# scrubbbbs/cbird

Measured on AMD Instinct MI355X. Metric: Hamming comparisons/sec + images hashed/sec, 1M-image index, 1/2/4/8 MI355X, higher is better.
Workload: dtype u64 hashes as 64 x FP4 signs, f32 accumulate (find, exact) / u8+f32 (hash)

## Files before the change

cbird_amd/csrc/hamm64_mfma.hip:

```cpp
#include <algorithm>
#include <mutex>
#include <vector>

#include "cbh_internal.h"
#include "fp4_sign.h"

namespace cbh {
namespace {

typedef _Float16 h2 __attribute__((ext_vector_type(2)));
typedef unsigned v4u_t __attribute__((ext_vector_type(4)));

constexpr int kThreads = 256;
constexpr int kWaves = 4;
constexpr int kHT = 8;
constexpr int kG = 2;
constexpr int e8m0(int e) { return (int)((uint32_t)(127 + e) * 0x01010101u); }

constexpr uint32_t kNeedlePad = 384;
constexpr uint32_t kNeedleBytes = 80;
struct NeedleScratch {
  uint32_t nq_pad;
  __host__ __device__ constexpr uint32_t words() const { return 0u; }
  __host__ __device__ constexpr uint32_t fold() const { return 2u * nq_pad; }
  __host__ __device__ constexpr uint32_t pre48() const { return 3u * nq_pad; }
  __host__ __device__ constexpr uint32_t pre16() const { return pre48() + nq_pad / 128u * 192u; }
  __host__ __device__ constexpr uint32_t total() const { return pre16() + nq_pad / 128u * 64u; }
};
static_assert(kNeedlePad % 64u == 0 && kNeedlePad % 96u == 0 && kNeedlePad % 128u == 0,
              "whole pairs, triples and quadruples of needle tiles");
static_assert(NeedleScratch{kNeedlePad}.total() * 16u == kNeedlePad * kNeedleBytes &&
                  NeedleScratch{5u * kNeedlePad}.total() * 16u == 5u * kNeedlePad * kNeedleBytes,
              "the regions add up to kNeedleBytes per padded needle");

__global__ __launch_bounds__(256) void k_expand_needles(const uint64_t* __restrict__ q, uint32_t nq,
                                                        uint32_t nq_pad, uint4* __restrict__ qx) {
  const uint32_t i = blockIdx.x * 256u + threadIdx.x;
  const NeedleScratch L{nq_pad};
  if (i >= L.total()) return;
  const uint32_t* w = reinterpret_cast<const uint32_t*>(q);
  if (i < L.fold()) {
    qx[i] = fp4_expand32((i >> 1) < nq ? w[i] : 0u);
  } else if (i < L.pre48()) {
    const uint32_t j = i - L.fold();
    qx[i] = fp4_expand32(j < nq ? w[2u * j] ^ w[2u * j + 1u] : 0u);
  } else if (i < L.pre16()) {
    const uint32_t u = i - L.pre48(), quad = u / 192u, m = (u % 192u) >> 6, c = u & 31u, kb = (u >> 5) & 1u;
    uint2 o[2];
#pragma unroll
    for (uint32_t k = 0; k < 2; ++k) {
      const uint32_t s = 2u * (2u * m + kb) + k, j = quad * 128u + (s / 3u) * 32u + c;
      const uint32_t lo = j < nq ? w[2u * j] : 0u, hi = j < nq ? w[2u * j + 1u] : 0u;
      o[k] = fp4_expand16(pre48_sub(lo, hi, s % 3u), s == 3u || s == 7u || s == 9u ? kFp4Four : kFp4Half);
    }
    qx[i] = make_uint4(o[0].x, o[0].y, o[1].x, o[1].y);
  } else {
    const uint32_t u = i - L.pre16(), c = u & 31u, kb = (u >> 5) & 1u;
    const uint32_t j0 = (u >> 6) * 128u + kb * 64u + c, j1 = j0 + 32u;
    const uint2 lo = fp4_expand16(j0 < nq ? fold16(w[2u * j0], w[2u * j0 + 1u]) : 0u, kFp4Half);
    const uint2 hi = fp4_expand16(j1 < nq ? fold16(w[2u * j1], w[2u * j1 + 1u]) : 0u, kFp4Four);
    qx[i] = make_uint4(lo.x, lo.y, hi.x, hi.y);
  }
}

__device__ __forceinline__ uint32_t as_u32(float f) { return __builtin_bit_cast(uint32_t, f); }
__device__ __forceinline__ void wave_order() {
  asm volatile("" ::: "memory");
  __builtin_amdgcn_wave_barrier();
  asm volatile("" ::: "memory");
}
__device__ __forceinline__ uint32_t wave_rank(uint64_t m, uint32_t base = 0u) {
  return __builtin_amdgcn_mbcnt_hi((uint32_t)(m >> 32), __builtin_amdgcn_mbcnt_lo((uint32_t)m, base));
}
__device__ __forceinline__ uint32_t cd_row(uint32_t g, uint32_t lane) { return (g & 3u) + 8u * (g >> 2) + 4u * (lane >> 5); }

struct HitParams {
  uint32_t thresh, n, nq, keep0;
  const uint64_t* q;
  const uint32_t* ids;
  cbh_record* rec;
  unsigned long long cap;
  unsigned long long* total;
  const uint2* hay;
  const uint2* qmask;
};

constexpr uint32_t kOutCap = 128;
__device__ __forceinline__ void out_flush(uint32_t* s_out, uint32_t& nout, const HitParams& hp) {
  if (nout == 0) return;
  wave_order();
  const uint32_t lane = threadIdx.x & 63u;
  unsigned long long base = 0;
  if (lane == 0) base = atomicAdd(hp.total, (unsigned long long)nout);
  const uint32_t blo = (uint32_t)__builtin_amdgcn_readfirstlane((int)(uint32_t)base);
  const uint32_t bhi = (uint32_t)__builtin_amdgcn_readfirstlane((int)(uint32_t)(base >> 32));
  base = ((unsigned long long)bhi << 32) | blo;
  for (uint32_t k = lane; k < nout; k += 64u) {
    const uint2 r = *reinterpret_cast<const uint2*>(&s_out[2u * k]);
    if (base + k < hp.cap) hp.rec[base + k] = ((cbh_record)r.y << 32) | r.x;
  }
  wave_order();
  nout = 0;
}
__device__ __forceinline__ void out_push(uint32_t* s_out, uint32_t& nout, bool has, uint32_t qidx, uint32_t dist,
                                         uint32_t id, const HitParams& hp) {
  const uint64_t m = __builtin_amdgcn_ballot_w64(has);
  if (m == 0) return;
  const uint32_t c = (uint32_t)__popcll(m);
  if (nout + c > kOutCap) out_flush(s_out, nout, hp);
  if (has) *reinterpret_cast<uint2*>(&s_out[2u * wave_rank(m, nout)]) = make_uint2(id, (qidx << 7) | dist);
  nout += c;
}

__device__ __forceinline__ bool mask_ok(const HitParams& hp, uint32_t row, uint32_t qi, uint64_t nv) {
  if (!hp.qmask) return true;
  const uint2 hv = hp.hay[row], mk = hp.qmask[qi];
  return (((hv.x ^ (uint32_t)nv) & mk.x) | ((hv.y ^ (uint32_t)(nv >> 32)) & mk.y)) == 0;
}
__device__ __forceinline__ void out_match(uint32_t* s_out, uint32_t& nout, bool under, uint32_t row, uint32_t qi,
                                          uint64_t nv, uint32_t dist, const HitParams& hp) {
  bool has = false;
  uint32_t id = 0;
  if (under && row < hp.n && mask_ok(hp, row, qi, nv)) {
    id = hp.ids[row];
    has = id != 0 || hp.keep0;
  }
  out_push(s_out, nout, has, qi, dist, id, hp);
}

template <int N, class Step>
__device__ __forceinline__ void needle_loop(const uint4* base, uint32_t voff, uint32_t nsteps, uint32_t last, Step&& step) {
  const __amdgpu_buffer_rsrc_t rsrc = __builtin_amdgcn_make_buffer_rsrc(const_cast<uint4*>(base), 0, (int)0xffffffffu, 0x27000);
  auto load = [&](uint32_t s, uint4 (&o)[N]) __attribute__((always_inline)) {
#pragma unroll
    for (uint32_t m = 0; m < (uint32_t)N; ++m) {
      const v4u_t v = __builtin_amdgcn_raw_buffer_load_b128(rsrc, (int)voff, (int)(min(s * N + m, last) * 1024u), 0);
      o[m] = make_uint4(v.x, v.y, v.z, v.w);
    }
  };
  uint4 x[N], y[N];
  load(0, x);
#pragma unroll 1
  for (uint32_t s = 0; s < nsteps; s += 2) {
    load(min(s + 1, nsteps - 1), y);
    step(s, x);
    if (s + 1 < nsteps) {
      load(min(s + 2, nsteps - 1), x);
      step(s + 1, y);
    }
  }
}
constexpr uint32_t kNoClamp = 0xffffffffu;

constexpr uint32_t kFlagMaskPre = (1u << 5) | (1u << 11) | (1u << 17) | (1u << 23);
constexpr uint32_t kFieldOnes = 1u + (1u << 6) + (1u << 12) + (1u << 18);

constexpr uint32_t kPendCap = 320;
constexpr uint32_t kOutOff = 2u * kPendCap;
constexpr uint32_t kItemOff = kOutOff + 2u * kOutCap;
constexpr uint32_t kItemCap = 63u + 64u * 8u;
constexpr uint32_t kPreQueue = kItemOff + kItemCap + 1u;
static_assert(kPendCap >= 63u + (kHT / kG) * 64u, "pending list: every lane of every group of a step");
static_assert(kG == 2, "a descriptor names the two reduction chains of a group of 32 registers");

template <int A, int B, int G>
__device__ __forceinline__ uint32_t or_regs(const v16f (&c)[G]) {
  static_assert(B - A >= 3, "range");
  uint32_t o = as_u32(c[A >> 4][A & 15]) | as_u32(c[(A + 1) >> 4][(A + 1) & 15]) | as_u32(c[(A + 2) >> 4][(A + 2) & 15]);
#pragma unroll
  for (int r = A + 3; r < B; r += 2)
    o |= as_u32(c[r >> 4][r & 15]) | (r + 1 < B ? as_u32(c[(r + 1) >> 4][(r + 1) & 15]) : 0u);
  return o;
}

#define CBH_SCALED_MFMA(A, B, C, SCALE_B) __builtin_amdgcn_mfma_scale_f32_32x32x64_f8f6f4(A, B, C, 4, 4, 0, kScaleOne, 0, SCALE_B)

struct Pre32 {
  static constexpr int kTiles = kHT, kOps = 2;
  static constexpr uint32_t operands(NeedleScratch L) { return L.fold(); }
  static __device__ __forceinline__ uint32_t last_op(uint32_t n_pairs, uint32_t p0) { return n_pairs - 1u - p0; }
  static __device__ __forceinline__ v8i hay(uint2 hv, uint32_t) { return fp4_operand(fp4_expand32(hv.x ^ hv.y)); }
  static __device__ __forceinline__ uint32_t bias(uint32_t t) { return 16u + (t - 1u); }
  static __device__ __forceinline__ int scale(int m, uint32_t half) {
    return m == 0 ? (half ? e8m0(5) : e8m0(-1)) : (half ? e8m0(17) : e8m0(11));
  }
  static __device__ __forceinline__ void chain(const v8i (&a)[kTiles], int t0, const v8i (&b)[kOps], const v16f& c0,
                                               const int (&sc)[kOps], v16f (&c)[kG]) {
#pragma unroll
    for (int t = 0; t < kG; ++t) c[t] = CBH_SCALED_MFMA(a[t0 + t], b[0], c0, sc[0]);
#pragma unroll
    for (int t = 0; t < kG; ++t) c[t] = CBH_SCALED_MFMA(a[t0 + t], b[1], c[t], sc[1]);
  }
};

struct Pre48 {
  static constexpr int kTiles = 6, kOps = 3;
  static constexpr uint32_t operands(NeedleScratch L) { return L.pre48(); }
  static __device__ __forceinline__ uint32_t last_op(uint32_t, uint32_t) { return kNoClamp; }
  static __device__ __forceinline__ v8i hay(uint2 hv, uint32_t half) {
    const uint32_t e0 = pre48_sub(hv.x, hv.y, 0), e1 = pre48_sub(hv.x, hv.y, 1), e2 = pre48_sub(hv.x, hv.y, 2);
    const uint2 s0 = fp4_expand16(half ? e2 : e0, kFp4Half);
    const uint2 s1 = fp4_expand16(half ? e0 : e1, half ? kFp4Four : kFp4Half);
    const uint2 s2 = fp4_expand16(half ? e1 : e2, kFp4Half);
    const uint2 s3 = fp4_expand16(half ? e2 : e0, half ? kFp4Half : kFp4Four);
    return v8i{(int)s0.x, (int)s0.y, (int)s1.x, (int)s1.y, (int)s2.x, (int)s2.y, (int)s3.x, (int)s3.y};
  }
  static __device__ __forceinline__ uint32_t bias(uint32_t t) { return 8u + t; }
  static __device__ __forceinline__ int scale(int m, uint32_t half) {
    return m == 0 ? e8m0(1) : m == 1 ? (half ? e8m0(10) : e8m0(7)) : (half ? e8m0(19) : e8m0(13));
  }
  static __device__ __forceinline__ void chain(const v8i (&a)[kTiles], int t0, const v8i (&b)[kOps], const v16f& c0,
                                               const int (&sc)[kOps], v16f (&c)[kG]) {
#pragma unroll
    for (int m = 0; m < kOps; ++m)
#pragma unroll
      for (int t = 0; t < kG; ++t) {
        const v8i& h = a[t0 + t];
        c[t] = CBH_SCALED_MFMA((v8i{h[2 * m], h[2 * m + 1], h[2 * m + 2], h[2 * m + 3], 0, 0, 0, 0}), b[m], m ? c[t] : c0, sc[m]);
      }
  }
};

struct Pre16 {
  static constexpr int kTiles = kHT, kOps = 1;
  static constexpr uint32_t operands(NeedleScratch L) { return L.pre16(); }
  static __device__ __forceinline__ uint32_t last_op(uint32_t, uint32_t) { return kNoClamp; }
  static __device__ __forceinline__ v8i hay(uint2 hv, uint32_t) {
    const uint32_t f = fold16(hv.x, hv.y);
    const uint2 s0 = fp4_expand16(f, kFp4Half), s1 = fp4_expand16(f, kFp4Four);
    return v8i{(int)s0.x, (int)s0.y, (int)s1.x, (int)s1.y, 0, 0, 0, 0};
  }
  static __device__ __forceinline__ uint32_t bias(uint32_t t) { return 24u + (t - 1u); }
  static __device__ __forceinline__ int scale(int, uint32_t half) { return half ? e8m0(13) : e8m0(1); }
  static __device__ __forceinline__ void chain(const v8i (&a)[kTiles], int t0, const v8i (&b)[kOps], const v16f& c0,
                                               const int (&sc)[kOps], v16f (&c)[kG]) {
#pragma unroll
    for (int t = 0; t < kG; ++t) c[t] = CBH_SCALED_MFMA(a[t0 + t], b[0], c0, sc[0]);
  }
};

#define CBH_MFMA_PARAMS                                                                                              \
  const uint2 *__restrict__ hay, const uint32_t *__restrict__ ids, uint32_t n, const uint64_t *__restrict__ q,       \
      const uint4 *__restrict__ qx, uint32_t nq, uint32_t n_pairs, uint32_t pairs_per_chunk, uint32_t thresh,        \
      cbh_record *__restrict__ rec, unsigned long long cap, unsigned long long *__restrict__ total, uint32_t keep0,  \
      const uint2 *__restrict__ qmask, const uint4 *__restrict__ qf
#define CBH_MFMA_ARGS hay, ids, n, q, qx, nq, n_pairs, pairs_per_chunk, thresh, rec, cap, total, keep0, qmask, qf

template <class V>
__device__ __forceinline__ void prefilter_body(CBH_MFMA_PARAMS) {
  constexpr int HT = V::kTiles, G = kG;
  __shared__ __attribute__((aligned(16))) uint32_t s_queue_[kWaves][kPreQueue];
  __shared__ __attribute__((aligned(16))) uint2 s_hay_[kWaves][HT * 32];
  const uint32_t lane = threadIdx.x & 63u;
  const uint32_t wave = (uint32_t)__builtin_amdgcn_readfirstlane((int)(threadIdx.x >> 6));
  const uint32_t r = lane & 31u, half = lane >> 5;
  const uint32_t tile0 = (blockIdx.x * kWaves + wave) * HT;
  if (tile0 * 32u >= n) return;
  uint32_t* s_queue = s_queue_[wave];
  uint2* s_hay = s_hay_[wave];
  uint32_t* s_out = s_queue + kOutOff;
  uint32_t nout = 0;

  v8i a[HT];
#pragma unroll
  for (int t = 0; t < HT; ++t) {
    const uint32_t row = (tile0 + t) * 32u + r;
    const uint2 hv = row < n ? hay[row] : make_uint2(0u, 0u);
    a[t] = V::hay(hv, half);
    if (half == 0) s_hay[t * 32 + r] = hv;
  }
  wave_order();
  v16f c0;
#pragma unroll
  for (int g = 0; g < 16; ++g) c0[g] = 8388608.0f + (float)(V::bias(thresh) * kFieldOnes);
  asm volatile("" : "+v"(c0));
  int scale[V::kOps];
#pragma unroll
  for (int m = 0; m < V::kOps; ++m) {
    scale[m] = V::scale(m, half);
    asm volatile("" : "+v"(scale[m]));
  }

  const uint32_t p0 = blockIdx.y * pairs_per_chunk;
  const uint32_t p1 = min(n_pairs, p0 + pairs_per_chunk);
  const HitParams hp = {thresh, n, nq, keep0, q, ids, rec, cap, total, hay, qmask};

  uint32_t npend = 0;
  uint32_t nitem = 0;
  uint32_t* s_item = s_queue + kItemOff;
  auto work = [&](uint32_t idx, bool live) {
    const uint32_t it = s_item[idx];
    const uint32_t f = it & 3u, ch = (it >> 2) & 1u, L = (it >> 3) & 63u, pp = p0 + 2u * (it >> 11);
    const uint32_t row0 = ((it >> 9) & 3u) * 64u;
    const uint32_t qi = pp * 64u + (L & 31u) + 32u * f;
    const uint64_t nv = live && qi < hp.nq ? hp.q[qi] : 0;
    const uint32_t qlo = (uint32_t)nv, qhi = (uint32_t)(nv >> 32);
    const uint32_t rows = nv == 0 ? 0u : ch ? 0xfffe0000u : 0x0001ffffu;
    const uint2* hq = s_hay + row0 + cd_row(16u * ch, L);
    uint32_t hit = 0;
#pragma unroll 1
    for (uint32_t i = 0; i < 5u; ++i) {
      const uint32_t qd = 4u * ch + i;
      const uint4* h4 = reinterpret_cast<const uint4*>(hq + 8u * min(i, 4u - ch));
      const uint4 x = h4[0], y = h4[1];
      const uint32_t d0 = __popc(x.x ^ qlo) + __popc(x.y ^ qhi), d1 = __popc(x.z ^ qlo) + __popc(x.w ^ qhi);
      const uint32_t d2 = __popc(y.x ^ qlo) + __popc(y.y ^ qhi), d3 = __popc(y.z ^ qlo) + __popc(y.w ^ qhi);
      const uint32_t m4 = (d0 < hp.thresh ? 1u : 0u) | (d1 < hp.thresh ? 2u : 0u) | (d2 < hp.thresh ? 4u : 0u) |
                          (d3 < hp.thresh ? 8u : 0u);
      hit |= qd < 8u ? m4 << (4u * qd) : 0u;
    }
    hit &= rows;
    while (__builtin_amdgcn_ballot_w64(hit != 0) != 0) {
      const uint32_t wr = row0 + cd_row((uint32_t)__builtin_ctz(hit | 0x80000000u), L);
      const uint2 hv = s_hay[wr];
      out_match(s_out, nout, hit != 0, tile0 * 32u + wr, qi, nv, __popc(hv.x ^ qlo) + __popc(hv.y ^ qhi), hp);
      hit &= hit - 1u;
    }
  };
  auto drain = [&](bool all) {
    wave_order();
    const uint32_t keep = all ? 0u : (npend & 63u);
    uint32_t k0 = keep;
    for (;;) {
      if (nitem < 64u && k0 < npend) {
        const uint2 e = *reinterpret_cast<const uint2*>(&s_queue[2u * min(k0 + lane, npend - 1u)]);
        uint32_t cm = 0;
#pragma unroll
        for (uint32_t c = 0; c < 2; ++c) {
          const uint32_t w = e.x >> c;
          cm |= (((w >> 23) & 1u) ? 0xfu : (((w >> 5) & 1u) | (((w >> 11) & 1u) << 1) | (((w >> 17) & 1u) << 2))) << (4u * c);
        }
        if (k0 + lane >= npend) cm = 0;
#pragma unroll
        for (uint32_t b = 0; b < 8; ++b) {
          const bool on = ((cm >> b) & 1u) != 0;
          const uint64_t m = __builtin_amdgcn_ballot_w64(on);
          if (on) s_item[wave_rank(m, nitem)] = (e.y << 3) | b;
          nitem += (uint32_t)__popcll(m);
        }
        k0 += 64u;
        wave_order();
        continue;
      }
      uint32_t idx;
      bool live = true;
      if (nitem >= 64u) {
        nitem -= 64u;
        idx = nitem + lane;
      } else if (all && nitem != 0) {
        idx = min(lane, nitem - 1u);
        live = lane < nitem;
        nitem = 0;
      } else {
        break;
      }
      work(idx, live);
      wave_order();
    }
    npend = keep;
  };

  auto detect = [&](const v16f (&c)[G], const uint32_t group, const uint32_t step) __attribute__((always_inline)) {
    constexpr int R = G * 16;
    constexpr int RA = R / 2 + 1;
    const uint32_t half0 = or_regs<0, RA, G>(c), half1 = or_regs<RA, R, G>(c);
    const uint32_t flags = (half0 | half1) & kFlagMaskPre;
    const uint64_t hm = __builtin_amdgcn_ballot_w64(flags != 0);
    if (hm != 0) {
      static_assert(R == 32, "two chains of 17 and 15 registers");
      uint32_t ln = lane;
      asm volatile("" : "+v"(ln));
      if (flags != 0)
        *reinterpret_cast<uint2*>(&s_queue[2u * wave_rank(hm, npend)]) =
            make_uint2((half0 & kFlagMaskPre) | ((half1 & kFlagMaskPre) << 1), ln | (group << 6) | (step << 8));
      npend += (uint32_t)__popcll(hm);
    }
  };

  needle_loop<V::kOps>(qf + (size_t)(p0 >> 1) * (V::kOps * 64u), lane * 16u, (p1 - p0 + 1u) >> 1, V::last_op(n_pairs, p0),
                       [&](const uint32_t s, const uint4 (&nn)[V::kOps]) __attribute__((always_inline)) {
    v8i b[V::kOps];
#pragma unroll
    for (int m = 0; m < V::kOps; ++m) b[m] = fp4_operand(nn[m]);
#pragma unroll
    for (int t0 = 0; t0 < HT; t0 += G) {
      v16f c[G];
      V::chain(a, t0, b, c0, scale, c);
      detect(c, (uint32_t)(t0 / G), s);
    }
    if (npend >= 64u) drain(false);
  });
  if (npend | nitem) drain(true);
  out_flush(s_out, nout, hp);
}

template <bool PRE>
__global__ void k_hamm64_mfma(CBH_MFMA_PARAMS);
template <>
__global__ __launch_bounds__(kThreads, 4) void k_hamm64_mfma<true>(CBH_MFMA_PARAMS) { prefilter_body<Pre32>(CBH_MFMA_ARGS); }
__global__ __launch_bounds__(kThreads, 3) void k_hamm64_mfma48(CBH_MFMA_PARAMS) { prefilter_body<Pre48>(CBH_MFMA_ARGS); }
__global__ __launch_bounds__(kThreads, 4) void k_hamm64_mfma16(CBH_MFMA_PARAMS) { prefilter_body<Pre16>(CBH_MFMA_ARGS); }

__device__ __forceinline__ void load_hay_words(const uint2* __restrict__ hay, uint32_t n, uint32_t tile0, v8i (&a)[kHT]) {
  const uint32_t r = threadIdx.x & 31u, half = (threadIdx.x >> 5) & 1u;
#pragma unroll
  for (int t = 0; t < kHT; ++t) {
    const uint32_t row = (tile0 + t) * 32u + r;
    const uint2 hv = row < n ? hay[row] : make_uint2(0u, 0u);
    a[t] = fp4_operand(fp4_expand32(half ? hv.y : hv.x));
  }
}

constexpr uint32_t kLoZero2 = 0x4080u, kHiZero2 = 0x4B40u;
__device__ __forceinline__ h2 as_h2(float f) { return __builtin_bit_cast(h2, f); }
__device__ __forceinline__ h2 pkmax3(h2 a, h2 b, h2 c) {
  return __builtin_elementwise_maximum(__builtin_elementwise_maximum(a, b), c);
}
__device__ __forceinline__ void handle_tile2(const v16f& c, uint32_t row0, uint32_t p, uint32_t lo_key, uint32_t hi_key,
                                             const HitParams& hp, uint32_t* s_queue, uint32_t* s_out, uint32_t& nout) {
  const uint32_t lane = threadIdx.x & 63u;
  {
    h2 m0 = {0, 0}, m1 = {0, 0};
#pragma unroll
    for (int g = 0; g < 16; g += 4) {
      m0 = pkmax3(m0, as_h2(c[g]), as_h2(c[g + 1]));
      m1 = pkmax3(m1, as_h2(c[g + 2]), as_h2(c[g + 3]));
    }
    const uint32_t tb = __builtin_bit_cast(uint32_t, __builtin_elementwise_maximum(m0, m1));
    if (__builtin_amdgcn_ballot_w64((tb << 16) >= lo_key || tb >= hi_key) == 0) return;
  }
  uint32_t cnt = 0;
#pragma unroll
  for (int g = 0; g < 16; ++g) {
    const uint32_t bits = as_u32(c[g]);
    const bool fh = bits >= hi_key;
    const bool fl = (bits << 16) >= lo_key;
    if (__builtin_amdgcn_ballot_w64(fh || fl) == 0) continue;
    const uint64_t mh = __builtin_amdgcn_ballot_w64(fh);
    if (fh) s_queue[wave_rank(mh, cnt)] = ((kHiZero2 - (bits >> 16)) << 12) | (1u << 10) | ((uint32_t)g << 6) | lane;
    cnt += (uint32_t)__popcll(mh);
    const uint64_t ml = __builtin_amdgcn_ballot_w64(fl);
    if (fl) s_queue[wave_rank(ml, cnt)] = (((kLoZero2 - (bits & 0xffffu)) >> 1) << 12) | ((uint32_t)g << 6) | lane;
    cnt += (uint32_t)__popcll(ml);
  }
  wave_order();
  for (uint32_t k0 = 0; k0 < cnt; k0 += 64u) {
    const uint32_t k = k0 + lane;
    const uint32_t e = s_queue[min(k, cnt - 1u)];
    const uint32_t src = e & 63u, g = (e >> 6) & 15u, field = (e >> 10) & 1u, d = e >> 12;
    const uint32_t row = row0 + cd_row(g, src);
    const uint32_t qi = p * 64u + field * 32u + (src & 31u);
    bool under = false;
    uint64_t nv = 0;
    if (k < cnt && row < hp.n && qi < hp.nq) {
      nv = hp.q[qi];
      under = nv != 0 && d < hp.thresh;
    }
    out_match(s_out, nout, under, row, qi, nv, d, hp);
  }
  wave_order();
}

template <>
__global__ __launch_bounds__(kThreads, 1) void k_hamm64_mfma<false>(CBH_MFMA_PARAMS) {
  constexpr int HT = kHT, G = kG;
  constexpr uint32_t kQueue = 2048;
  __shared__ uint32_t s_queue_[kWaves][kQueue];
  __shared__ uint32_t s_out_[kWaves][2 * kOutCap];
  const uint32_t lane = threadIdx.x & 63u, wave = threadIdx.x >> 6;
  const uint32_t tile0 = (blockIdx.x * kWaves + wave) * HT;
  if (tile0 * 32u >= n) return;
  uint32_t* s_queue = s_queue_[wave];
  uint32_t* s_out = s_out_[wave];
  uint32_t nout = 0;

  v8i a[HT];
  load_hay_words(hay, n, tile0, a);
  v16f c0;
#pragma unroll
  for (int g = 0; g < 16; ++g) c0[g] = 8388608.0f + 16448.0f + 2097152.0f;
  asm volatile("" : "+v"(c0));
  const uint32_t lo_key = (kLoZero2 - 2u * (thresh - 1u)) << 16, hi_key = (kHiZero2 - (thresh - 1u)) << 16;
  const HitParams hp = {thresh, n, nq, keep0, q, ids, rec, cap, total, hay, qmask};

  const uint32_t p0 = blockIdx.y * pairs_per_chunk;
  const uint32_t p1 = min(n_pairs, p0 + pairs_per_chunk);
  needle_loop<2>(qx + (size_t)p0 * 128u, (2u * (lane & 31u) + (lane >> 5)) * 16u, p1 - p0, kNoClamp,
                 [&](const uint32_t s, const uint4 (&nn)[2]) __attribute__((always_inline)) {
    const v8i bA = fp4_operand(nn[0]), bB = fp4_operand(nn[1]);
#pragma unroll
    for (int t0 = 0; t0 < HT; t0 += G) {
      v16f c[G];
#pragma unroll
      for (int t = 0; t < G; ++t) c[t] = CBH_SCALED_MFMA(a[t0 + t], bA, c0, kScaleOne);
#pragma unroll
      for (int t = 0; t < G; ++t) c[t] = CBH_SCALED_MFMA(a[t0 + t], bB, c[t], e8m0(15));
      h2 m0 = {0, 0}, m1 = {0, 0};
#pragma unroll
      for (int t = 0; t < G; ++t)
#pragma unroll
        for (int g = 0; g < 16; g += 4) {
          m0 = pkmax3(m0, as_h2(c[t][g]), as_h2(c[t][g + 1]));
          m1 = pkmax3(m1, as_h2(c[t][g + 2]), as_h2(c[t][g + 3]));
        }
      const uint32_t mb = __builtin_bit_cast(uint32_t, __builtin_elementwise_maximum(m0, m1));
      if (__builtin_amdgcn_ballot_w64((mb << 16) >= lo_key || mb >= hi_key) != 0) {
#pragma unroll
        for (int t = 0; t < G; ++t)
          handle_tile2(c[t], (tile0 + t0 + t) * 32u, p0 + s, lo_key, hi_key, hp, s_queue, s_out, nout);
      }
    }
  });
  out_flush(s_out, nout, hp);
}
#undef CBH_MFMA_PARAMS
#undef CBH_MFMA_ARGS

constexpr uint32_t kFlagMask3 = (1u << 7) | (1u << 14) | (1u << 21);

__device__ __forceinline__ void handle_tile3(const v16f& c, uint32_t row0, uint32_t p3, const HitParams& hp,
                                             uint32_t* s_queue, uint32_t* s_out, uint32_t& nout) {
  const uint32_t lane = threadIdx.x & 63u;
  uint32_t any = 0;
#pragma unroll
  for (int g = 0; g < 16; ++g) any |= as_u32(c[g]);
  if (__builtin_amdgcn_ballot_w64((any & kFlagMask3) != 0) == 0) return;
  const uint32_t b = hp.thresh - 1u;
#pragma unroll 1
  for (uint32_t f = 0; f < 3; ++f) {
    uint32_t cnt = 0;
#pragma unroll
    for (int g = 0; g < 16; ++g) {
      const uint32_t bits = as_u32(c[g]);
      const bool fl = (bits >> (7u + 7u * f)) & 1u;
      const uint64_t m = __builtin_amdgcn_ballot_w64(fl);
      if (m == 0) continue;
      if (fl)
        s_queue[wave_rank(m, cnt)] = ((64u + b - ((bits >> (1u + 7u * f)) & 0x7fu)) << 12) | (f << 10) | ((uint32_t)g << 6) | lane;
      cnt += (uint32_t)__popcll(m);
    }
    wave_order();
    for (uint32_t k0 = 0; k0 < cnt; k0 += 64u) {
      const uint32_t k = k0 + lane;
      const uint32_t e = s_queue[min(k, cnt - 1u)];
      const uint32_t src = e & 63u, g = (e >> 6) & 15u, field = (e >> 10) & 3u, d = e >> 12;
      const uint32_t row = row0 + cd_row(g, src);
      const uint32_t qi = p3 * 96u + field * 32u + (src & 31u);
      const uint64_t nv = (k < cnt && row < hp.n && qi < hp.nq) ? hp.q[qi] : 0;
      out_match(s_out, nout, nv != 0, row, qi, nv, d, hp);
    }
    wave_order();
  }
}
// ... 250 lines not shown
```

cbird_amd/csrc/hamm64_scan.hip:

```cpp
#include <atomic>

#include "cbh_internal.h"

namespace cbh {
namespace {

constexpr int kThreads = 256;
constexpr int kH = 8;
constexpr int kQB = 8;

__device__ __forceinline__ uint32_t min3u(uint32_t a, uint32_t b, uint32_t c) {
  return min(min(a, b), c);
}

__device__ __forceinline__ void emit(cbh_record* __restrict__ rec, unsigned long long cap,
                                     unsigned long long* __restrict__ total, uint32_t qidx,
                                     uint32_t dist, uint32_t id) {
  unsigned long long slot = atomicAdd(total, 1ull);
  if (slot < cap) rec[slot] = ((cbh_record)qidx << 39) | ((cbh_record)dist << 32) | id;
}

template <int H>
__device__ __forceinline__ void exact_block(const uint2 (&h)[H], uint32_t base_idx, uint32_t n,
                                            const uint32_t* __restrict__ ids,
// ... 114 lines not shown
        asm volatile("v_mov_b32 %0, %1" : "=v"(ql[i]) : "s"(cur[i].x));
        if (MODE == MODE_FULL) asm volatile("v_mov_b32 %0, %1" : "=v"(qh[i]) : "s"(cur[i].y));
      }
      uint32_t x[QB][H];
      __builtin_amdgcn_sched_barrier(0);
#pragma unroll
      for (int i = 0; i < QB; ++i)
#pragma unroll
        for (int j = 0; j < H; ++j) x[i][j] = h[j].x ^ ql[i];
      __builtin_amdgcn_sched_barrier(0);
      if (MODE == MODE_FULL) {
#pragma unroll
        for (int i = 0; i < QB; ++i)
#pragma unroll
          for (int j = 0; j < H; ++j) x[i][j] = (uint32_t)__popc(x[i][j]);
        uint32_t y[QB][H];
        __builtin_amdgcn_sched_barrier(0);
#pragma unroll
        for (int i = 0; i < QB; ++i)
#pragma unroll
          for (int j = 0; j < H; ++j) y[i][j] = h[j].y ^ qh[i];
        __builtin_amdgcn_sched_barrier(0);
#pragma unroll
        for (int i = 0; i < QB; i += 2)
#pragma unroll
          for (int j = 0; j < H; ++j)
            acc[j] = min3u(acc[j], x[i][j] + (uint32_t)__popc(y[i][j]),
                           x[i + 1][j] + (uint32_t)__popc(y[i + 1][j]));
      } else {
#pragma unroll
        for (int i = 0; i < QB; i += 2)
#pragma unroll
          for (int j = 0; j < H; ++j)
            acc[j] = min3u(acc[j], (uint32_t)__popc(x[i][j]), (uint32_t)__popc(x[i + 1][j]));
      }
      __builtin_amdgcn_sched_barrier(0);
      uint32_t m = acc[0];
#pragma unroll
      for (int j = 1; j + 1 < H; j += 2) m = min3u(m, acc[j], acc[j + 1]);
      if (H % 2 == 0) m = min(m, acc[H - 1]);
      if (m < thresh) refine_block<H, QB>(h, acc, cur, base_idx, n, ids, qb, thresh, rec, cap, total, keep0, qmask);
    }
#pragma unroll
    for (int i = 0; i < QB; ++i) cur[i] = nxt[i];
  }
  if (qb < q1) exact_block<H>(h, base_idx, n, ids, q, qb, q1, thresh, rec, cap, total, keep0, qmask);
}

__global__ __launch_bounds__(256) void k_zero_needle_list(const uint64_t* __restrict__ q, uint32_t nq,
                                                          uint32_t* __restrict__ list ) {
  const uint32_t qi = blockIdx.x * 256u + threadIdx.x;
  if (qi < nq && q[qi] == 0) list[1u + atomicAdd(&list[0], 1u)] = qi;
}

__global__ __launch_bounds__(256) void k_zero_needle_scan(const uint2* __restrict__ hay, const uint32_t* __restrict__ ids,
                                                          uint32_t n, const uint32_t* __restrict__ list, uint32_t thresh,
                                                          cbh_record* __restrict__ rec, unsigned long long cap,
                                                          unsigned long long* __restrict__ total, uint32_t keep0,
                                                          const uint2* __restrict__ qmask) {
  const uint32_t i = blockIdx.x * 256u + threadIdx.x;
  const uint32_t nz = list[0];
  if (i >= n || nz == 0) return;
  const uint2 h = hay[i];
  const uint32_t d = (uint32_t)__popc(h.x) + (uint32_t)__popc(h.y);
  if (d >= thresh) return;
  const uint32_t id = ids[i];
  if (id == 0 && !keep0) return;
  for (uint32_t k = 0; k < nz; ++k) {
    const uint32_t qi = list[1u + k];
    const uint2 mk = qmask ? qmask[qi] : make_uint2(0u, 0u);
    if (((h.x & mk.x) | (h.y & mk.y)) == 0) emit(rec, cap, total, qi, d, id);
  }
}

constexpr unsigned kLoneSlots = 8;
__global__ __launch_bounds__(256) void k_find_one(const uint2* __restrict__ hay, const uint32_t* __restrict__ ids,
                                                  uint32_t n, uint32_t qlo, uint32_t qhi, uint32_t thresh,
                                                  unsigned* __restrict__ d_state, LoneBlock* __restrict__ host,
                                                  unsigned long long seq) {
  const uint32_t base = blockIdx.x * (256u * kLoneSlots) + threadIdx.x;
  bool wrote = false;
#pragma unroll
  for (unsigned k = 0; k < kLoneSlots; ++k) {
    const uint32_t i = base + k * 256u;
    if (i >= n) break;
    const uint2 hv = hay[i];
    const uint32_t d = (uint32_t)__popc(hv.x ^ qlo) + (uint32_t)__popc(hv.y ^ qhi);
    if (d < thresh) {
      const uint32_t id = ids[i];
      if (id != 0) {
        const unsigned slot = atomicAdd(&d_state[0], 1u);
        if (slot < LoneBlock::kRecs) {
          host->recs[slot] = ((cbh_record)d << 32) | id;
          wrote = true;
        }
      }
    }
  }
  if (wrote) __threadfence_system();
  __syncthreads();
  if (threadIdx.x == 0) {
    __threadfence();
    if (atomicAdd(&d_state[1], 1u) == gridDim.x - 1u) {
      __threadfence();
      host->count = atomicExch(&d_state[0], 0u);
      d_state[1] = 0u;
      __threadfence_system();
      __hip_atomic_store(const_cast<unsigned long long*>(&host->done), seq, __ATOMIC_RELEASE, __HIP_MEMORY_SCOPE_SYSTEM);
    }
  }
}

}

int launch_find_one(const uint64_t* d_hashes, const uint32_t* d_ids, size_t n, uint64_t q, int thresh, unsigned* d_state,
                    LoneBlock* h_block, unsigned long long seq, hipStream_t stream) {
  if (n == 0 || n > 0xfffffff0ull || !d_state || !h_block || thresh <= 0) return CBH_E_INVAL;
  const unsigned per_wg = 256u * kLoneSlots;
  hipLaunchKernelGGL(k_find_one, dim3((unsigned)((n + per_wg - 1) / per_wg)), dim3(256), 0, stream,
                     reinterpret_cast<const uint2*>(d_hashes), d_ids, (uint32_t)n, (uint32_t)q, (uint32_t)(q >> 32),
                     (uint32_t)thresh, d_state, h_block, seq);
  CBH_HIP(hipGetLastError());
  return CBH_OK;
}

int wait_find_one(const LoneBlock* h_block, unsigned long long seq, hipStream_t stream) {
  const unsigned long long* flag = const_cast<const unsigned long long*>(&h_block->done);
  for (unsigned spins = 0;; ++spins) {
    if (__atomic_load_n(flag, __ATOMIC_ACQUIRE) == seq) return CBH_OK;
    if ((spins & 0xfffu) == 0xfffu) {
      const hipError_t q = hipStreamQuery(stream);
      if (q == hipSuccess) {
        return __atomic_load_n(flag, __ATOMIC_ACQUIRE) == seq ? CBH_OK : CBH_E_HIP;
      }
      if (q != hipErrorNotReady) {
        set_last_error("k_find_one", q);
        return CBH_E_HIP;
      }
    }
#if defined(__x86_64__)
    __builtin_ia32_pause();
#endif
  }
}

namespace {

constexpr int kPreMax = 7;
constexpr size_t kMfmaMinNq = 256;
constexpr size_t kMfmaMinN = 4096;
constexpr int kPreStatic = 6;
constexpr double kTrueWeight = 8.0;
constexpr double kSlopePre = 1.3e4, kBaseFull = 15.75, kTrueFull = 2.7e5, kTruePre = 0.7e5;
constexpr double kBasePre = 8.55, kBase48 = 14.0, kSlope48 = 2.8e4, kTrue48 = 1.0e5, kPre48Margin = 0.9;
constexpr double kBase16 = 5.85, kPre16Margin = 0.9;
constexpr uint64_t kProbeMinPairs = 1ull << 31;

int g_scan_mfma = 1;
int g_pre_max_thresh = -1;
int g_pre_rate_max_e9 = 300000;
int g_pre48 = -1;
int g_pre16 = -1;
std::atomic<uint64_t> g_variant_mask[4];
std::atomic<uint64_t> g_n_probe{0};
std::atomic<long long> g_last_rate_e9{-1};
std::atomic<long long> g_last_true_e9{-1};
std::atomic<long long> g_last_rate48_e9{-1};
std::atomic<long long> g_last_rate16_e9{-1};

enum class Join { None, IfCheaper, Forced };
enum class Kernel { PopcEq, PopcPre, PopcFull, Mfma };
struct Route {
  Join join;
  Kernel kernel;
  double scan_ms;
};

Route route(size_t n, size_t nq, int thresh, bool masked) {
  Route r;
  const double pairs = (double)n * (double)nq;
  const double pre_ms = pairs * (thresh <= 5 ? 8.7e-12 : thresh == 6 ? 9.7e-12 : thresh == 7 ? 12.1e-12 : 15.8e-12);
  r.scan_ms = thresh == 1 ? pairs * 6.1e-12 : pre_ms;
  const bool joinable = thresh <= kJoinMaxThresh && !masked && n < 0xfffffff0ull;
  r.join = !joinable ? Join::None : g_scan_mfma == 4 ? Join::Forced
           : g_scan_mfma == 3 && pre_ms >= 1.0 ? Join::IfCheaper : Join::None;
  const bool mfma = thresh <= 65 && (g_scan_mfma == 2 || g_scan_mfma == 4 ||
                                     (g_scan_mfma != 0 && nq >= kMfmaMinNq && n >= kMfmaMinN));
  r.kernel = mfma ? Kernel::Mfma : thresh == 1 ? Kernel::PopcEq : thresh <= kPreMax ? Kernel::PopcPre : Kernel::PopcFull;
  return r;
}

void note_variant(int thresh, ScanVariant v) {
  for (int i = 1; i < 4; ++i)
    if (i == (int)v) g_variant_mask[i] |= 1ull << thresh; else g_variant_mask[i] &= ~(1ull << thresh);
}

int launch_popc(Kernel kernel, const uint64_t* d_hashes, const uint32_t* d_ids, size_t n, const uint64_t* d_q, size_t nq,
                int thresh, cbh_record* d_rec, size_t cap, unsigned long long* d_total, hipStream_t stream,
                const ScanOpts& o) {
  const uint32_t tile = kThreads * kH;
  const uint32_t tiles = (uint32_t)((n + tile - 1) / tile);
  const uint32_t q_chunk = scan_chunk(tiles, nq, 16384, 1024, kQB);
  dim3 grid(tiles, (uint32_t)((nq + q_chunk - 1) / q_chunk)), block(kThreads);
  const uint2* hay = reinterpret_cast<const uint2*>(d_hashes);
#define CBH_SCAN(MODE)                                                                                                  \
  hipLaunchKernelGGL((k_hamm64_scan<kH, kQB, MODE>), grid, block, 0, stream, hay, d_ids, (uint32_t)n, d_q, (uint32_t)nq, \
                     q_chunk, (uint32_t)thresh, d_rec, (unsigned long long)cap, d_total, (uint32_t)o.keep_id0,            \
                     reinterpret_cast<const uint2*>(o.d_qmask))
  if (kernel == Kernel::PopcEq) CBH_SCAN(MODE_EQ);
  else if (kernel == Kernel::PopcPre) CBH_SCAN(MODE_PRE);
  else CBH_SCAN(MODE_FULL);
#undef CBH_SCAN
  CBH_HIP(hipGetLastError());
  return CBH_OK;
}

}

bool scan_takes_mfma(size_t n, size_t nq, int thresh) {
  return thresh >= 1 && route(n, nq, thresh, false).kernel == Kernel::Mfma;
}

bool scan_routes_to_join(size_t n, size_t nq, int thresh, bool masked) {
  return thresh >= 1 && n >= 1 && nq >= 1 && route(n, nq, thresh, masked).join != Join::None;
}

ScanVariant scan_pick_pre(const uint64_t* d_hashes, size_t n, size_t n_total, const uint64_t* d_q, size_t nq, int thresh,
                          hipStream_t stream) {
  using V = ScanVariant;
  if (g_pre16 == 1 && thresh <= max_thresh(V::Pre16)) return V::Pre16;
  if (g_pre48 == 1 && thresh <= max_thresh(V::Pre48)) return V::Pre48;
  if (thresh > max_thresh(V::Pre32)) return V::Full;
  if (g_pre_max_thresh >= 0) return thresh <= g_pre_max_thresh ? V::Pre32 : V::Full;
  if (thresh > kProbeMaxThresh) return V::Full;
  double r_cand = 0, r_true = 0, r48 = 0, r16 = 0;
  if ((uint64_t)n_total * (uint64_t)nq < kProbeMinPairs ||
      !probe_fold_rates(d_hashes, n, d_q, nq, thresh, stream, &r_cand, &r_true, &r48, &r16))
    return thresh <= kPreStatic ? V::Pre32 : V::Full;
  g_last_rate_e9 = (long long)(r_cand * 1e9);
  g_last_true_e9 = (long long)(r_true * 1e9);
  g_last_rate48_e9 = (long long)(r48 * 1e9);
  g_last_rate16_e9 = (long long)(r16 * 1e9);
  g_n_probe++;
  const double d_pre = kSlopePre * (r_cand - kTrueWeight * r_true - (double)g_pre_rate_max_e9 * 1e-9);
  const bool pre = d_pre <= 0;
  const double t_pre = kBasePre + kSlopePre * r_cand + kTruePre * r_true, t_full = kBaseFull + kTrueFull * r_true;
  if (g_pre16 != 0 && pre && thresh <= max_thresh(V::Pre16) &&
      kBase16 + kSlopePre * r16 + kTruePre * r_true < kPre16Margin * t_pre)
    return V::Pre16;
  if (g_pre48 != 0) {
    const double t_48 = kBase48 + kSlope48 * r48 + kTrue48 * r_true;
    if (pre ? t_48 < kPre48Margin * t_pre : t_48 < t_full) return V::Pre48;
  }
  return pre ? V::Pre32 : V::Full;
}

namespace {

int launch_zero_needles(const uint64_t* d_hashes, const uint32_t* d_ids, size_t n, const uint64_t* d_q, size_t nq,
                        int thresh, cbh_record* d_rec, size_t cap, unsigned long long* d_total, hipStream_t stream,
                        const ScanOpts& o) {
  Scratch scratch(stream);
  uint32_t* list = nullptr;
  CBH_HIP(scratch.get(&list, (nq + 1) * sizeof(uint32_t)));
  CBH_HIP(hipMemsetAsync(list, 0, sizeof(uint32_t), stream));
  hipLaunchKernelGGL(k_zero_needle_list, dim3((unsigned)((nq + 255) / 256)), dim3(256), 0, stream, d_q, (uint32_t)nq, list);
  hipLaunchKernelGGL(k_zero_needle_scan, dim3((unsigned)((n + 255) / 256)), dim3(256), 0, stream,
                     reinterpret_cast<const uint2*>(d_hashes), d_ids, (uint32_t)n, list, (uint32_t)thresh, d_rec,
                     (unsigned long long)cap, d_total, (uint32_t)o.keep_id0, reinterpret_cast<const uint2*>(o.d_qmask));
  CBH_HIP(hipGetLastError());
  return CBH_OK;
}

int scan_nonzero_needles(const uint64_t* d_hashes, const uint32_t* d_ids, size_t n, const uint64_t* d_q, size_t nq,
                         int thresh, cbh_record* d_rec, size_t cap, unsigned long long* d_total, hipStream_t stream,
                         const ScanOpts& o);

}

int launch_hamm64_scan(const uint64_t* d_hashes, const uint32_t* d_ids, size_t n, const uint64_t* d_q, size_t nq,
                       int thresh, cbh_record* d_rec, size_t cap, unsigned long long* d_total, hipStream_t stream,
                       const ScanOpts& o) {
  if (n == 0 || nq == 0 || thresh <= 0) return CBH_OK;
  if (n > 0xfffffff0ull || nq > CBH_MAX_QUERIES_PER_CALL) return CBH_E_INVAL;
  const int rc = scan_nonzero_needles(d_hashes, d_ids, n, d_q, nq, thresh, d_rec, cap, d_total, stream, o);
  if (rc || !o.zero_needles) return rc;
  return launch_zero_needles(d_hashes, d_ids, n, d_q, nq, thresh, d_rec, cap, d_total, stream, o);
}

namespace {

int scan_nonzero_needles(const uint64_t* d_hashes, const uint32_t* d_ids, size_t n, const uint64_t* d_q, size_t nq,
                         int thresh, cbh_record* d_rec, size_t cap, unsigned long long* d_total, hipStream_t stream,
                         const ScanOpts& o) {
  const Route r = route(n, nq, thresh, o.d_qmask != nullptr);
  if (r.join != Join::None) {
    const bool force = r.join == Join::Forced;
    const int rc = launch_hamm64_join(d_hashes, d_ids, n, d_q, nq, thresh, d_rec, cap, d_total, stream, o, force, r.scan_ms);
    if (rc == CBH_OK || force || (rc != CBH_E_UNSUPPORTED && rc != CBH_E_NOMEM)) return rc;
    if (rc == CBH_E_NOMEM) cbh_clear_error();
  }
  if (r.kernel != Kernel::Mfma) return launch_popc(r.kernel, d_hashes, d_ids, n, d_q, nq, thresh, d_rec, cap, d_total, stream, o);
  const ScanVariant v = o.pre != ScanVariant::Auto ? o.pre : scan_pick_pre(d_hashes, n, n, d_q, nq, thresh, stream);
  if (thresh < 64) note_variant(thresh, v);
  return launch_hamm64_scan_mfma(d_hashes, d_ids, n, d_q, nq, thresh, d_rec, cap, d_total, stream, v, o);
}

// ... 33 lines not shown
```

Before: 86790 billion.

## Widen Pre48 prefilter to eight tiles and repack its hay operand sub-blocks

The Pre48 prefilter now processes eight haystack tiles per step instead of six, with tile count, group size and occupancy exposed as compile-time knobs. The pending-queue layout is generalised so descriptors can name more groups. The hay operand packing and needle sub-block order are rearranged so the middle MFMA reads a contiguous half and the outer ones share the low half, with matching scale exponents. The cost model's Pre48 base cost is lowered so the router picks this variant more often. Risks are more register pressure at the same launch bound and a possible correctness slip in the reordered sub-block and scale mapping.

Result: no change. 87150 billion (median of 6 runs) (+0.4%).

```diff
diff --git a/cbird_amd/csrc/hamm64_mfma.hip b/cbird_amd/csrc/hamm64_mfma.hip
--- a/cbird_amd/csrc/hamm64_mfma.hip
+++ b/cbird_amd/csrc/hamm64_mfma.hip
@@ -32,6 +32,7 @@
 static_assert(NeedleScratch{kNeedlePad}.total() * 16u == kNeedlePad * kNeedleBytes &&
                   NeedleScratch{5u * kNeedlePad}.total() * 16u == 5u * kNeedlePad * kNeedleBytes,
               "the regions add up to kNeedleBytes per padded needle");
+constexpr uint64_t kPre48Sub = 0x43ull | 0x05ull << 8 | 0x21ull << 16 | 0x87ull << 24 | 0xa9ull << 32 | 0x6bull << 40;
 
 __global__ __launch_bounds__(256) void k_expand_needles(const uint64_t* __restrict__ q, uint32_t nq,
                                                         uint32_t nq_pad, uint4* __restrict__ qx) {
@@ -49,9 +50,9 @@
     uint2 o[2];
 #pragma unroll
     for (uint32_t k = 0; k < 2; ++k) {
-      const uint32_t s = 2u * (2u * m + kb) + k, j = quad * 128u + (s / 3u) * 32u + c;
+      const uint32_t s = (uint32_t)(kPre48Sub >> (8u * (2u * m + kb) + 4u * k)) & 15u, j = quad * 128u + (s / 3u) * 32u + c;
       const uint32_t lo = j < nq ? w[2u * j] : 0u, hi = j < nq ? w[2u * j + 1u] : 0u;
-      o[k] = fp4_expand16(pre48_sub(lo, hi, s % 3u), s == 3u || s == 7u || s == 9u ? kFp4Four : kFp4Half);
+      o[k] = fp4_expand16(pre48_sub(lo, hi, s % 3u), s == 5u || s == 11u ? kFp4Four : kFp4Half);
     }
     qx[i] = make_uint4(o[0].x, o[0].y, o[1].x, o[1].y);
   } else {
@@ -155,13 +156,18 @@
 constexpr uint32_t kFlagMaskPre = (1u << 5) | (1u << 11) | (1u << 17) | (1u << 23);
 constexpr uint32_t kFieldOnes = 1u + (1u << 6) + (1u << 12) + (1u << 18);
 
-constexpr uint32_t kPendCap = 320;
-constexpr uint32_t kOutOff = 2u * kPendCap;
-constexpr uint32_t kItemOff = kOutOff + 2u * kOutCap;
 constexpr uint32_t kItemCap = 63u + 64u * 8u;
-constexpr uint32_t kPreQueue = kItemOff + kItemCap + 1u;
-static_assert(kPendCap >= 63u + (kHT / kG) * 64u, "pending list: every lane of every group of a step");
-static_assert(kG == 2, "a descriptor names the two reduction chains of a group of 32 registers");
+struct PreQueue {
+  uint32_t groups;
+  constexpr uint32_t pend_cap() const { return 64u + groups * 64u; }
+  constexpr uint32_t out_off() const { return 2u * pend_cap(); }
+  constexpr uint32_t item_off() const { return out_off() + 2u * kOutCap; }
+  constexpr uint32_t words() const { return item_off() + kItemCap + 1u; }
+  constexpr uint32_t group_bits() const { return groups <= 4u ? 2u : 3u; }
+};
+static_assert(PreQueue{4}.pend_cap() == 320u && PreQueue{4}.words() == 1472u && PreQueue{4}.group_bits() == 2u,
+              "four groups per step (Pre32, Pre16): the list as it was");
+static_assert(PreQueue{6}.pend_cap() >= 63u + 6u * 64u, "pending list: every lane of every group of a step");
 
 template <int A, int B, int G>
 __device__ __forceinline__ uint32_t or_regs(const v16f (&c)[G]) {
@@ -176,7 +182,7 @@
 #define CBH_SCALED_MFMA(A, B, C, SCALE_B) __builtin_amdgcn_mfma_scale_f32_32x32x64_f8f6f4(A, B, C, 4, 4, 0, kScaleOne, 0, SCALE_B)
 
 struct Pre32 {
-  static constexpr int kTiles = kHT, kOps = 2;
+  static constexpr int kTiles = kHT, kGroup = 2, kOps = 2;
   static constexpr uint32_t operands(NeedleScratch L) { return L.fold(); }
   static __device__ __forceinline__ uint32_t last_op(uint32_t n_pairs, uint32_t p0) { return n_pairs - 1u - p0; }
   static __device__ __forceinline__ v8i hay(uint2 hv, uint32_t) { return fp4_operand(fp4_expand32(hv.x ^ hv.y)); }
@@ -185,44 +191,56 @@
     return m == 0 ? (half ? e8m0(5) : e8m0(-1)) : (half ? e8m0(17) : e8m0(11));
   }
   static __device__ __forceinline__ void chain(const v8i (&a)[kTiles], int t0, const v8i (&b)[kOps], const v16f& c0,
-                                               const int (&sc)[kOps], v16f (&c)[kG]) {
-#pragma unroll
-    for (int t = 0; t < kG; ++t) c[t] = CBH_SCALED_MFMA(a[t0 + t], b[0], c0, sc[0]);
-#pragma unroll
-    for (int t = 0; t < kG; ++t) c[t] = CBH_SCALED_MFMA(a[t0 + t], b[1], c[t], sc[1]);
+                                               const int (&sc)[kOps], v16f (&c)[kGroup]) {
+#pragma unroll
+    for (int t = 0; t < kGroup; ++t) c[t] = CBH_SCALED_MFMA(a[t0 + t], b[0], c0, sc[0]);
+#pragma unroll
+    for (int t = 0; t < kGroup; ++t) c[t] = CBH_SCALED_MFMA(a[t0 + t], b[1], c[t], sc[1]);
   }
 };
 
+#ifndef CBH_PRE48_TILES
+#define CBH_PRE48_TILES 8
+#endif
+#ifndef CBH_PRE48_GROUP
+#define CBH_PRE48_GROUP 2
+#endif
+#ifndef CBH_PRE48_WAVES
+#define CBH_PRE48_WAVES 3
+#endif
 struct Pre48 {
-  static constexpr int kTiles = 6, kOps = 3;
+  static constexpr int kTiles = CBH_PRE48_TILES, kGroup = CBH_PRE48_GROUP, kOps = 3;
+  static constexpr int kWavesPerSimd = CBH_PRE48_WAVES;
+  static_assert((kGroup == 1 || kGroup == 2) && kTiles % kGroup == 0 && kTiles / kGroup <= 8 && kTiles <= kHT,
+                "whole groups of 16 or 32 accumulator registers; a descriptor has three bits for the group");
   static constexpr uint32_t operands(NeedleScratch L) { return L.pre48(); }
   static __device__ __forceinline__ uint32_t last_op(uint32_t, uint32_t) { return kNoClamp; }
   static __device__ __forceinline__ v8i hay(uint2 hv, uint32_t half) {
     const uint32_t e0 = pre48_sub(hv.x, hv.y, 0), e1 = pre48_sub(hv.x, hv.y, 1), e2 = pre48_sub(hv.x, hv.y, 2);
-    const uint2 s0 = fp4_expand16(half ? e2 : e0, kFp4Half);
-    const uint2 s1 = fp4_expand16(half ? e0 : e1, half ? kFp4Four : kFp4Half);
-    const uint2 s2 = fp4_expand16(half ? e1 : e2, kFp4Half);
-    const uint2 s3 = fp4_expand16(half ? e2 : e0, half ? kFp4Half : kFp4Four);
-    return v8i{(int)s0.x, (int)s0.y, (int)s1.x, (int)s1.y, (int)s2.x, (int)s2.y, (int)s3.x, (int)s3.y};
+    const uint2 x0 = fp4_expand16(half ? e2 : e0, half ? kFp4Four : kFp4Half);
+    const uint2 x1 = fp4_expand16(half ? e0 : e1, kFp4Half);
+    const uint2 y0 = fp4_expand16(e1, kFp4Half), y1 = fp4_expand16(e2, kFp4Half);
+    return v8i{(int)x0.x, (int)x0.y, (int)x1.x, (int)x1.y, (int)y0.x, (int)y0.y, (int)y1.x, (int)y1.y};
   }
   static __device__ __forceinline__ uint32_t bias(uint32_t t) { return 8u + t; }
   static __device__ __forceinline__ int scale(int m, uint32_t half) {
-    return m == 0 ? e8m0(1) : m == 1 ? (half ? e8m0(10) : e8m0(7)) : (half ? e8m0(19) : e8m0(13));
+    return m == 0 ? (half ? e8m0(1) : e8m0(7)) : m == 1 ? (half ? e8m0(13) : e8m0(1)) : (half ? e8m0(13) : e8m0(19));
   }
   static __device__ __forceinline__ void chain(const v8i (&a)[kTiles], int t0, const v8i (&b)[kOps], const v16f& c0,
-                                               const int (&sc)[kOps], v16f (&c)[kG]) {
+                                               const int (&sc)[kOps], v16f (&c)[kGroup]) {
 #pragma unroll
     for (int m = 0; m < kOps; ++m)
 #pragma unroll
-      for (int t = 0; t < kG; ++t) {
+      for (int t = 0; t < kGroup; ++t) {
         const v8i& h = a[t0 + t];
-        c[t] = CBH_SCALED_MFMA((v8i{h[2 * m], h[2 * m + 1], h[2 * m + 2], h[2 * m + 3], 0, 0, 0, 0}), b[m], m ? c[t] : c0, sc[m]);
+        const int o = m == 1 ? 4 : 0;
+        c[t] = CBH_SCALED_MFMA((v8i{h[o], h[o + 1], h[o + 2], h[o + 3], 0, 0, 0, 0}), b[m], m ? c[t] : c0, sc[m]);
       }
   }
 };
 
 struct Pre16 {
-  static constexpr int kTiles = kHT, kOps = 1;
+  static constexpr int kTiles = kHT, kGroup = 2, kOps = 1;
   static constexpr uint32_t operands(NeedleScratch L) { return L.pre16(); }
   static __device__ __forceinline__ uint32_t last_op(uint32_t, uint32_t) { return kNoClamp; }
   static __device__ __forceinline__ v8i hay(uint2 hv, uint32_t) {
@@ -233,9 +251,9 @@
   static __device__ __forceinline__ uint32_t bias(uint32_t t) { return 24u + (t - 1u); }
   static __device__ __forceinline__ int scale(int, uint32_t half) { return half ? e8m0(13) : e8m0(1); }
   static __device__ __forceinline__ void chain(const v8i (&a)[kTiles], int t0, const v8i (&b)[kOps], const v16f& c0,
-                                               const int (&sc)[kOps], v16f (&c)[kG]) {
-#pragma unroll
-    for (int t = 0; t < kG; ++t) c[t] = CBH_SCALED_MFMA(a[t0 + t], b[0], c0, sc[0]);
+                                               const int (&sc)[kOps], v16f (&c)[kGroup]) {
+#pragma unroll
+    for (int t = 0; t < kGroup; ++t) c[t] = CBH_SCALED_MFMA(a[t0 + t], b[0], c0, sc[0]);
   }
 };
 
@@ -248,8 +266,12 @@
 
 template <class V>
 __device__ __forceinline__ void prefilter_body(CBH_MFMA_PARAMS) {
-  constexpr int HT = V::kTiles, G = kG;
-  __shared__ __attribute__((aligned(16))) uint32_t s_queue_[kWaves][kPreQueue];
+  constexpr int HT = V::kTiles, G = V::kGroup;
+  constexpr int R = G * 16, RA = R / 2 + 1;
+  constexpr PreQueue Q{(uint32_t)(HT / G)};
+  constexpr uint32_t kOutOff = Q.out_off(), kItemOff = Q.item_off(), GB = Q.group_bits();
+  static_assert((G == 1 || G == 2) && HT % G == 0, "a descriptor names the two reduction chains of a group of 16 or 32 registers");
+  __shared__ __attribute__((aligned(16))) uint32_t s_queue_[kWaves][Q.words()];
   __shared__ __attribute__((aligned(16))) uint2 s_hay_[kWaves][HT * 32];
   const uint32_t lane = threadIdx.x & 63u;
   const uint32_t wave = (uint32_t)__builtin_amdgcn_readfirstlane((int)(threadIdx.x >> 6));
@@ -290,24 +312,25 @@
   uint32_t* s_item = s_queue + kItemOff;
   auto work = [&](uint32_t idx, bool live) {
     const uint32_t it = s_item[idx];
-    const uint32_t f = it & 3u, ch = (it >> 2) & 1u, L = (it >> 3) & 63u, pp = p0 + 2u * (it >> 11);
-    const uint32_t row0 = ((it >> 9) & 3u) * 64u;
+    const uint32_t f = it & 3u, ch = (it >> 2) & 1u, L = (it >> 3) & 63u, pp = p0 + 2u * (it >> (9u + GB));
+    const uint32_t row0 = ((it >> 9) & ((1u << GB) - 1u)) * (uint32_t)(G * 32);
     const uint32_t qi = pp * 64u + (L & 31u) + 32u * f;
     const uint64_t nv = live && qi < hp.nq ? hp.q[qi] : 0;
     const uint32_t qlo = (uint32_t)nv, qhi = (uint32_t)(nv >> 32);
-    const uint32_t rows = nv == 0 ? 0u : ch ? 0xfffe0000u : 0x0001ffffu;
-    const uint2* hq = s_hay + row0 + cd_row(16u * ch, L);
+    constexpr uint32_t QH = (uint32_t)R / 8u, kRows0 = (1u << RA) - 1u, kRows1 = (uint32_t)((1ull << R) - 1ull) & ~kRows0;
+    const uint32_t rows = nv == 0 ? 0u : ch ? kRows1 : kRows0;
+    const uint2* hq = s_hay + row0 + cd_row(QH * 4u * ch, L);
     uint32_t hit = 0;
 #pragma unroll 1
-    for (uint32_t i = 0; i < 5u; ++i) {
-      const uint32_t qd = 4u * ch + i;
-      const uint4* h4 = reinterpret_cast<const uint4*>(hq + 8u * min(i, 4u - ch));
+    for (uint32_t i = 0; i < QH + 1u; ++i) {
+      const uint32_t qd = QH * ch + i;
+      const uint4* h4 = reinterpret_cast<const uint4*>(hq + 8u * min(i, QH - ch));
       const uint4 x = h4[0], y = h4[1];
       const uint32_t d0 = __popc(x.x ^ qlo) + __popc(x.y ^ qhi), d1 = __popc(x.z ^ qlo) + __popc(x.w ^ qhi);
       const uint32_t d2 = __popc(y.x ^ qlo) + __popc(y.y ^ qhi), d3 = __popc(y.z ^ qlo) + __popc(y.w ^ qhi);
       const uint32_t m4 = (d0 < hp.thresh ? 1u : 0u) | (d1 < hp.thresh ? 2u : 0u) | (d2 < hp.thresh ? 4u : 0u) |
                           (d3 < hp.thresh ? 8u : 0u);
-      hit |= qd < 8u ? m4 << (4u * qd) : 0u;
+      hit |= qd < 2u * QH ? m4 << (4u * qd) : 0u;
     }
     hit &= rows;
     while (__builtin_amdgcn_ballot_w64(hit != 0) != 0) {
@@ -361,18 +384,15 @@
   };
 
   auto detect = [&](const v16f (&c)[G], const uint32_t group, const uint32_t step) __attribute__((always_inline)) {
-    constexpr int R = G * 16;
-    constexpr int RA = R / 2 + 1;
     const uint32_t half0 = or_regs<0, RA, G>(c), half1 = or_regs<RA, R, G>(c);
     const uint32_t flags = (half0 | half1) & kFlagMaskPre;
     const uint64_t hm = __builtin_amdgcn_ballot_w64(flags != 0);
     if (hm != 0) {
-      static_assert(R == 32, "two chains of 17 and 15 registers");
       uint32_t ln = lane;
       asm volatile("" : "+v"(ln));
       if (flags != 0)
         *reinterpret_cast<uint2*>(&s_queue[2u * wave_rank(hm, npend)]) =
-            make_uint2((half0 & kFlagMaskPre) | ((half1 & kFlagMaskPre) << 1), ln | (group << 6) | (step << 8));
+            make_uint2((half0 & kFlagMaskPre) | ((half1 & kFlagMaskPre) << 1), ln | (group << 6) | (step << (6u + GB)));
       npend += (uint32_t)__popcll(hm);
     }
   };
@@ -398,7 +418,7 @@
 __global__ void k_hamm64_mfma(CBH_MFMA_PARAMS);
 template <>
 __global__ __launch_bounds__(kThreads, 4) void k_hamm64_mfma<true>(CBH_MFMA_PARAMS) { prefilter_body<Pre32>(CBH_MFMA_ARGS); }
-__global__ __launch_bounds__(kThreads, 3) void k_hamm64_mfma48(CBH_MFMA_PARAMS) { prefilter_body<Pre48>(CBH_MFMA_ARGS); }
+__global__ __launch_bounds__(kThreads, Pre48::kWavesPerSimd) void k_hamm64_mfma48(CBH_MFMA_PARAMS) { prefilter_body<Pre48>(CBH_MFMA_ARGS); }
 __global__ __launch_bounds__(kThreads, 4) void k_hamm64_mfma16(CBH_MFMA_PARAMS) { prefilter_body<Pre16>(CBH_MFMA_ARGS); }
 
 __device__ __forceinline__ void load_hay_words(const uint2* __restrict__ hay, uint32_t n, uint32_t tile0, v8i (&a)[kHT]) {
diff --git a/cbird_amd/csrc/hamm64_scan.hip b/cbird_amd/csrc/hamm64_scan.hip
--- a/cbird_amd/csrc/hamm64_scan.hip
+++ b/cbird_amd/csrc/hamm64_scan.hip
@@ -290,7 +290,7 @@
 constexpr int kPreStatic = 6;
 constexpr double kTrueWeight = 8.0;
 constexpr double kSlopePre = 1.3e4, kBaseFull = 15.75, kTrueFull = 2.7e5, kTruePre = 0.7e5;
-constexpr double kBasePre = 8.55, kBase48 = 14.0, kSlope48 = 2.8e4, kTrue48 = 1.0e5, kPre48Margin = 0.9;
+constexpr double kBasePre = 8.55, kBase48 = 13.2, kSlope48 = 2.8e4, kTrue48 = 1.0e5, kPre48Margin = 0.9;
 constexpr double kBase16 = 5.85, kPre16Margin = 0.9;
 constexpr uint64_t kProbeMinPairs = 1ull << 31;
 
```
